# JonasGeiping/fullbatchtraining

Hardware: AMD Instinct MI355X
Metric: full-batch GD images/sec (ResNet-18 CIFAR-10 shaped, all chunks accumulated per step) (higher is better)
Workload: dtype bf16

## Files before the change

### fullbatchtraining_amd/csrc/conv_igemm.hip

```cpp
#include "common.h"
#include "profile.h"

#include "conv_params.h"

template <typename T, int BN_CO>
__global__ __launch_bounds__(256) void conv_igemm_kernel(const ConvParams p) {
    constexpr int EB = ET<T>::EB;
    constexpr int BKE = 128 / EB;
    constexpr int WROWS = BN_CO / 32;
    constexpr int FI = BN_CO / 32;
    constexpr int FJ = 4;
    constexpr int TILE_CHUNKS = (128 + BN_CO) * 8;
    __shared__ uint4 lds[2 * TILE_CHUNKS];

    const int tid = threadIdx.x, lane = tid & 63, wave = tid >> 6;
    const int wave_co = wave >> 1, wave_px = wave & 1;
    const int mblk = blockIdx.x, co_blk = blockIdx.y, cls = blockIdx.z;
    const int cpy = (p.os == 2) ? (cls >> 1) : 0, cpx = (p.os == 2) ? (cls & 1) : 0;
    const int chunk = tid & 7, lrow = tid >> 3;

    int a_img[4], a_y[4], a_x[4];
    const int qHW = p.qH * p.qW;
#pragma unroll
    for (int i = 0; i < 4; ++i) {
        const int m = mblk * 128 + lrow + 32 * i;
        if (m < p.M) {
            const int n = m / qHW, rem = m - n * qHW, qy = rem / p.qW, qx = rem - qy * p.qW;
            a_img[i] = n * p.Hs * p.Ws; a_y[i] = qy * p.ss; a_x[i] = qx * p.ss;
        } else {
            a_img[i] = 0; a_y[i] = -(1 << 28); a_x[i] = 0;
        }
    }
    const int first_img = (mblk * 128) / qHW;
    const char* wbase = p.wgt + (long long)(first_img / p.imgs_per_wset) * p.wset_stride_bytes;
    const int taps = p.R * p.S;
    const long long wrow_bytes = (long long)taps * p.Cs * EB;
    const char* wptr[WROWS];
#pragma unroll
    for (int i = 0; i < WROWS; ++i) wptr[i] = wbase + (long long)(co_blk * BN_CO + lrow + 32 * i) * wrow_bytes + chunk * 16;

    auto tap_valid = [&](int t, int& dy, int& dx) -> bool {
        const int r = t / p.S, s = t - r * p.S;
        if (p.mode == 0) { dy = r - p.pad; dx = s - p.pad; return true; }
        if (p.os == 1) { dy = p.pad - r; dx = p.pad - s; return true; }
        const int vy = cpy + p.pad - r, vx = cpx + p.pad - s;
        if ((vy & 1) || (vx & 1)) return false;
        dy = vy >> 1; dx = vx >> 1;
        return true;
    };
    const int kc = (p.Cs + BKE - 1) / BKE;
    int n_valid = 0;
    for (int t = 0; t < taps; ++t) { int dy, dx; n_valid += tap_valid(t, dy, dx) ? 1 : 0; }
    const int n_iter = n_valid * kc;

    uint4 ra[4], rw[WROWS];
    int cur_t = -1, cur_c = kc, cur_dy = 0, cur_dx = 0;
    auto advance = [&]() {
        if (++cur_c >= kc) {
            cur_c = 0;
            do { ++cur_t; } while (cur_t < taps && !tap_valid(cur_t, cur_dy, cur_dx));
        }
    };
    auto gload = [&]() {
        const int c0 = cur_c * BKE;
        const bool cvalid = c0 + chunk * ET<T>::VEC < p.Cs;
#pragma unroll
        for (int i = 0; i < 4; ++i) {
            const int sy = a_y[i] + cur_dy, sx = a_x[i] + cur_dx;
            const bool ok = cvalid && (unsigned)sy < (unsigned)p.Hs && (unsigned)sx < (unsigned)p.Ws;
            ra[i] = make_uint4(0, 0, 0, 0);
            if (ok) ra[i] = *(const uint4*)(p.src + ((long long)(a_img[i] + sy * p.Ws + sx) * p.Cs + c0) * EB + chunk * 16);
        }
#pragma unroll
        for (int i = 0; i < WROWS; ++i) {
            rw[i] = make_uint4(0, 0, 0, 0);
            if (cvalid) rw[i] = *(const uint4*)(wptr[i] + ((long long)cur_t * p.Cs + c0) * EB);
        }
    };
    auto lstore = [&](int buf) {
        uint4* base = lds + buf * TILE_CHUNKS;
#pragma unroll
        for (int i = 0; i < 4; ++i) { const int row = lrow + 32 * i; base[row * 8 + (chunk ^ (row & 7))] = ra[i]; }
#pragma unroll
        for (int i = 0; i < WROWS; ++i) { const int row = 128 + lrow + 32 * i; base[row * 8 + (chunk ^ (row & 7))] = rw[i]; }
    };

    f32x4_t acc[FI][FJ];
#pragma unroll
    for (int i = 0; i < FI; ++i)
#pragma unroll
        for (int j = 0; j < FJ; ++j) acc[i][j] = (f32x4_t){0.f, 0.f, 0.f, 0.f};

    if (n_iter > 0) {
        advance(); gload(); lstore(0);
        __syncthreads();
        for (int it = 0; it < n_iter; ++it) {
            const int buf = it & 1;
            const bool more = it + 1 < n_iter;
            if (more) { advance(); gload(); }
            const uint4* base = lds + buf * TILE_CHUNKS;
#pragma unroll
            for (int h = 0; h < 2; ++h) {
                const int pc = ((lane >> 4) + 4 * h) ^ (lane & 7);
                uint4 wf[FI], pf[FJ];
#pragma unroll
                for (int i = 0; i < FI; ++i) wf[i] = base[(128 + wave_co * (BN_CO / 2) + i * 16 + (lane & 15)) * 8 + pc];
#pragma unroll
                for (int j = 0; j < FJ; ++j) pf[j] = base[(wave_px * 64 + j * 16 + (lane & 15)) * 8 + pc];
#pragma unroll
                for (int i = 0; i < FI; ++i)
#pragma unroll
                    for (int j = 0; j < FJ; ++j) acc[i][j] = mma_chunk<T>(wf[i], pf[j], acc[i][j]);
            }
            if (more) lstore(buf ^ 1);
            __syncthreads();
        }
    }

    float ssum[FI][4], ssq[FI][4];
#pragma unroll
    for (int i = 0; i < FI; ++i)
#pragma unroll
        for (int r = 0; r < 4; ++r) { ssum[i][r] = 0.f; ssq[i][r] = 0.f; }
#pragma unroll
    for (int j = 0; j < FJ; ++j) {
        const int m = mblk * 128 + wave_px * 64 + j * 16 + (lane & 15);
        if (m < p.M) {
            const int n = m / qHW, rem = m - n * qHW, qy = rem / p.qW, qx = rem - qy * p.qW;
            const int oy = qy * p.os + cpy, ox = qx * p.os + cpx;
            const long long pix = ((long long)n * p.Hd + oy) * p.Wd + ox;
#pragma unroll
            for (int i = 0; i < FI; ++i) {
                const int co = co_blk * BN_CO + wave_co * (BN_CO / 2) + i * 16 + (lane >> 4) * 4;
                float v[4] = {acc[i][j][0], acc[i][j][1], acc[i][j][2], acc[i][j][3]};
                if (p.addend_mode == 1) {
                    const char* ap = p.addend + (pix * p.Cd + co) * EB;
                    if constexpr (EB == 4) { const float4 a = *(const float4*)ap; v[0] += a.x; v[1] += a.y; v[2] += a.z; v[3] += a.w; }
                    else { const uint2 a = *(const uint2*)ap; v[0] += __uint_as_float(a.x << 16); v[1] += __uint_as_float(a.x & 0xffff0000u);
                           v[2] += __uint_as_float(a.y << 16); v[3] += __uint_as_float(a.y & 0xffff0000u); }
                } else if (p.addend_mode == 2) {
                    const long long apix = ((long long)n * (p.Hd >> 1) + (oy >> 1)) * (p.Wd >> 1) + (ox >> 1);
                    const char* ap = p.addend + (apix * p.Cd + co) * EB;
                    if constexpr (EB == 4) { const float4 a = *(const float4*)ap; v[0] += 0.25f * a.x; v[1] += 0.25f * a.y; v[2] += 0.25f * a.z; v[3] += 0.25f * a.w; }
                    else { const uint2 a = *(const uint2*)ap; v[0] += 0.25f * __uint_as_float(a.x << 16); v[1] += 0.25f * __uint_as_float(a.x & 0xffff0000u);
                           v[2] += 0.25f * __uint_as_float(a.y << 16); v[3] += 0.25f * __uint_as_float(a.y & 0xffff0000u); }
                }
                char* dp = p.dst + (pix * p.Cd + co) * EB;
                if constexpr (EB == 4) *(float4*)dp = make_float4(v[0], v[1], v[2], v[3]);
                else *(uint2*)dp = make_uint2(pack_bf16x2(v[0], v[1]), pack_bf16x2(v[2], v[3]));
#pragma unroll
                for (int r = 0; r < 4; ++r) { ssum[i][r] += v[r]; ssq[i][r] += v[r] * v[r]; }
            }
        }
    }
    if (p.stat != nullptr) {
        float* red = (float*)lds;
        __syncthreads();
#pragma unroll
        for (int i = 0; i < FI; ++i)
#pragma unroll
            for (int r = 0; r < 4; ++r) {
                float a = ssum[i][r], b = ssq[i][r];
                a = row16_sum(a); b = row16_sum(b);
                if ((lane & 15) == 0) {
                    const int col = wave_co * (BN_CO / 2) + i * 16 + (lane >> 4) * 4 + r;
                    red[(wave_px * BN_CO + col) * 2] = a; red[(wave_px * BN_CO + col) * 2 + 1] = b;
                }
            }
        __syncthreads();
        if (tid < BN_CO) {
            const float a = red[tid * 2] + red[(BN_CO + tid) * 2];
            const float b = red[tid * 2 + 1] + red[(BN_CO + tid) * 2 + 1];
            const long long blk = (long long)cls * gridDim.x + mblk;
            p.stat[blk * p.Cd + co_blk * BN_CO + tid] = a;
            p.stat[((long long)p.n_mblocks + blk) * p.Cd + co_blk * BN_CO + tid] = b;
        }
    }
}

int fb_try_conv3x3_halo4(const fb_conv_args* a, hipStream_t st);
int fb_try_conv3x3_halo5(const fb_conv_args* a, hipStream_t st);
int fb_conv3x3_halo5_takes(const fb_conv_args* a);
int fb_try_conv3x3s2_dgrad_quad(const fb_conv_args* a, hipStream_t st);
int fb_try_conv1x1_k32(const fb_conv_args* a, hipStream_t st);
int fb_try_conv1x1_stream(const fb_conv_args* a, hipStream_t st);
int fb_try_conv1x1_gemm(const fb_conv_args* a, hipStream_t st);
int fb_try_conv1x1_pipe(const fb_conv_args* a, hipStream_t st);

int fb_conv1x1_pipe_takes(const fb_conv_args* a);
int fb_conv3x3_halo4_takes(const fb_conv_args* a);
int fb_conv1x1_gemm_takes(const fb_conv_args* a);
static int igemm_masked_addend_ok(const fb_conv_args* a) {
    if (getenv("FB_IGEMM_NO_MASK") != nullptr || a->mode != 1 || a->stride != 1 || a->bst_x) return 0;
    if (a->Cs % 32 != 0 || a->Cd % 64 != 0) return 0;
    static const bool v1 = getenv("FB_IGEMM_V1") != nullptr;
    if (v1) return 0;
    ConvParams p{};
    p.n_img = a->n_img; p.Hs = a->Hs; p.Ws = a->Ws; p.Cs = a->Cs; p.Hd = a->Hd; p.Wd = a->Wd; p.Cd = a->Cd; p.R = a->R; p.S = a->S;
    p.qH = a->Hd; p.qW = a->Wd;
    return fb_igemm_glds_fits(p, a->dtype);
}
extern "C" int32_t fb_conv_masked_addend_supported(const fb_conv_args* a) {
    if (!a || !a->addend || !a->addend_mask || a->addend_mode != 1) return 0;
    return fb_conv3x3_halo5_takes(a) || fb_conv1x1_pipe_takes(a) || fb_conv3x3_halo4_takes(a) || fb_conv1x1_gemm_takes(a) || igemm_masked_addend_ok(a);
}

extern "C" int32_t fb_conv_bwd_stat_supported(const fb_conv_args* a) {
    static const bool disabled = getenv("FB_DISABLE_FUSED_BWD_STAT") != nullptr;
    if (disabled || !a || !a->bst_x || !a->bst_mask || !a->stat_partial || a->mode != 1 || a->dtype != FB_BF16) return 0;
    if ((long long)a->n_img * a->Hd * a->Wd % 128 != 0) return 0;
    static const char* widths = getenv("FB_FUSED_BWD_STAT_W");
    if (widths) {
        char tag[8];
        snprintf(tag, sizeof(tag), "%d,", a->Wd);
        char list[64];
        snprintf(list, sizeof(list), "%s,", widths);
        if (!strstr(list, tag) || (a->Wd < 10 && list != strstr(list, tag) && *(strstr(list, tag) - 1) != ',')) return 0;
    }
    return fb_conv3x3_halo5_takes(a) || fb_conv3x3_halo4_takes(a);
}

template <typename T> static int launch_conv(const ConvParams& p, int classes, hipStream_t st) {
    const int mblocks = (p.M + 127) / 128;
    if (p.Cd % 128 == 0 && (long long)mblocks * (p.Cd / 128) * classes >= 512) {
        dim3 grid(mblocks, p.Cd / 128, classes);
        hipLaunchKernelGGL((conv_igemm_kernel<T, 128>), grid, dim3(256), 0, st, p);
    } else {
        dim3 grid(mblocks, p.Cd / 64, classes);
        hipLaunchKernelGGL((conv_igemm_kernel<T, 64>), grid, dim3(256), 0, st, p);
    }
    return 0;
}

extern "C" int fb_conv2d(const fb_conv_args* a, void* stream) {
    if (!a || !a->src || !a->wgt || !a->dst) FB_FAIL(FB_ERR_ARG, "fb_conv2d: null pointer");
    const int EB = a->dtype == FB_F32 ? 4 : 2;
    if (a->Cs % 32 != 0) FB_FAIL(FB_ERR_SHAPE, "fb_conv2d: Cs=%d must be a multiple of 32", a->Cs);
    if (a->Cd % 64 != 0) FB_FAIL(FB_ERR_SHAPE, "fb_conv2d: Cd=%d must be a multiple of 64", a->Cd);
    if (a->mode != 0 && a->mode != 1) FB_FAIL(FB_ERR_ARG, "fb_conv2d: mode %d", a->mode);
    if (a->addend_mask && !fb_conv_masked_addend_supported(a))
        FB_FAIL(FB_ERR_UNSUPPORTED, "fb_conv2d: addend_mask is not implemented for this shape (ask fb_conv_masked_addend_supported)");
    if (a->bst_x && !fb_conv_bwd_stat_supported(a))
        FB_FAIL(FB_ERR_UNSUPPORTED, "fb_conv2d: the fused BatchNorm-backward reduction is not implemented for this shape (ask fb_conv_bwd_stat_supported)");
    if (a->stride != 1 && a->stride != 2) FB_FAIL(FB_ERR_UNSUPPORTED, "fb_conv2d: stride %d", a->stride);
    ConvParams p;
    p.src = (const char*)a->src; p.wgt = (const char*)a->wgt; p.dst = (char*)a->dst; p.addend = (const char*)a->addend;
    p.stat = a->stat_partial;
    p.n_img = a->n_img; p.Hs = a->Hs; p.Ws = a->Ws; p.Cs = a->Cs; p.Hd = a->Hd; p.Wd = a->Wd; p.Cd = a->Cd;
    p.R = a->R; p.S = a->S; p.stride = a->stride; p.pad = a->pad; p.mode = a->mode;
    p.imgs_per_wset = a->imgs_per_wset > 0 ? a->imgs_per_wset : a->n_img;
    p.wset_stride_bytes = a->wset_stride * EB;
    p.addend_mode = a->addend ? a->addend_mode : 0;
    p.addend_mask = a->addend ? (const unsigned char*)a->addend_mask : nullptr;
    p.amax_src = a->dtype == FB_F32 ? a->amax_src : nullptr; p.amax_wgt = a->dtype == FB_F32 ? a->amax_wgt : nullptr;
    if ((p.amax_src == nullptr) != (p.amax_wgt == nullptr)) FB_FAIL(FB_ERR_ARG, "fb_conv2d: amax_src and amax_wgt go together");
    p.amax_imgs = a->amax_imgs > 0 ? a->amax_imgs : a->n_img;
    int classes = 1;
    if (a->mode == 0) {
        if (a->Hd != (a->Hs + 2 * a->pad - a->R) / a->stride + 1 || a->Wd != (a->Ws + 2 * a->pad - a->S) / a->stride + 1)
            FB_FAIL(FB_ERR_SHAPE, "fb_conv2d: fwd output %dx%d inconsistent with input %dx%d", a->Hd, a->Wd, a->Hs, a->Ws);
        p.qH = a->Hd; p.qW = a->Wd; p.os = 1; p.ss = a->stride;
    } else {
        if (a->Hs != (a->Hd + 2 * a->pad - a->R) / a->stride + 1 || a->Ws != (a->Wd + 2 * a->pad - a->S) / a->stride + 1)
            FB_FAIL(FB_ERR_SHAPE, "fb_conv2d: dgrad shapes inconsistent");
        if (a->stat_partial && !a->bst_x) FB_FAIL(FB_ERR_ARG, "fb_conv2d: statistics in mode 1 need bst_x / bst_mask");
        if (a->stride == 1) { p.qH = a->Hd; p.qW = a->Wd; p.os = 1; }
        else {
            if ((a->Hd & 1) || (a->Wd & 1)) FB_FAIL(FB_ERR_SHAPE, "fb_conv2d: stride-2 dgrad needs even input dims");
            p.qH = a->Hd / 2; p.qW = a->Wd / 2; p.os = 2; classes = 4;
        }
        p.ss = 1;
    }
    p.M = a->n_img * p.qH * p.qW;
    p.n_mblocks = ((p.M + 127) / 128) * classes;
    hipStream_t st = (hipStream_t)stream;
    const int32_t info[FB_PROF_INFO] = {a->n_img, a->Hs, a->Ws, a->Cs, a->Hd, a->Wd, a->Cd, a->R, a->stride,
                                        (a->addend ? a->addend_mode : 0) | (a->addend_mask ? 4 : 0) | (a->bst_x ? 8 : 0) | (a->dtype << 4), 0};
    const int prof = fb_prof_begin(a->mode == 0 ? FB_PROF_IGEMM_FWD : FB_PROF_IGEMM_DGRAD, st, info);
    static const bool v1 = getenv("FB_IGEMM_V1") != nullptr;
    int kernel = 0;
    if (fb_try_conv1x1_k32(a, st)) kernel = FB_K_CONV1X1_K32;
    else if ((a->mode == 0 || a->addend) && (a->Cs == 256 || a->Cs == 128) && fb_try_conv1x1_gemm(a, st)) kernel = FB_K_CONV1X1_GEMM;
    else if (fb_try_conv1x1_pipe(a, st)) kernel = FB_K_CONV1X1_PIPE;
    else if (fb_try_conv1x1_stream(a, st)) kernel = FB_K_CONV1X1_STREAM;
    else if (fb_try_conv1x1_gemm(a, st)) kernel = FB_K_CONV1X1_GEMM;
    else if (fb_try_conv3x3s2_dgrad_quad(a, st)) kernel = FB_K_S2_DGRAD_QUAD;
    else if (fb_try_conv3x3_halo5(a, st)) kernel = FB_K_HALO5;
    else if (fb_try_conv3x3_halo4(a, st)) kernel = FB_K_HALO4;
    else {
        p.zeros = nullptr;
        kernel = FB_K_IGEMM_GLDS;
        if (v1 || !fb_launch_igemm_glds(p, classes, a->dtype, st)) {
            if (p.addend_mask) FB_FAIL(FB_ERR_UNSUPPORTED, "fb_conv2d: the register-staged implicit GEMM does not apply addend_mask (tensor beyond 2^31 bytes per tile or FB_IGEMM_V1)");
            if (p.amax_src) FB_FAIL(FB_ERR_UNSUPPORTED, "fb_conv2d: the register-staged implicit GEMM has no fp16x2 path (tensor beyond 2^31 bytes or FB_IGEMM_V1)");
            if (a->dtype == FB_F32) launch_conv<float>(p, classes, st); else launch_conv<bf16_tag>(p, classes, st);
            kernel = FB_K_IGEMM_V1;
        }
    }
    fb_prof_kernel(prof, kernel);
    fb_prof_end(prof, st);
    FB_CHECK_LAUNCH("fb_conv2d");
    return FB_OK;
}
```

Baseline: 216,100.

## Add persistent halo-staged kernel for stride-2 3x3 forward conv 64->128

Adds a specialised persistent kernel for the ResNet-18 stride-2 3x3 forward convolution (32x32x64 to 16x16x128, bf16). Weights stay resident in registers, the input halo is loaded straight into LDS through buffer loads and double-buffered so the next tile prefetches during the current tile's MFMA work. BN statistics are fused into the epilogue. It replaces the generic implicit-GEMM path for this one layer shape, which can lower load traffic and launch overhead, at the cost of heavy register pressure and code tied to one shape. FB_K_S2_FWD is used but not defined in the shown code.

```diff
diff --git a/fullbatchtraining_amd/csrc/conv3x3s2_fwd.hip b/fullbatchtraining_amd/csrc/conv3x3s2_fwd.hip
--- /dev/null
+++ b/fullbatchtraining_amd/csrc/conv3x3s2_fwd.hip
@@ -0,0 +1,215 @@
+#include "common.h"
+
+#include <type_traits>
+
+struct S2FwdParams {
+    const char* src; const char* wgt; char* dst; float* stat;
+    int n_tiles;
+};
+
+namespace {
+template <int N> __device__ __forceinline__ void s2_wait_lgkmcnt() {
+    asm volatile("s_waitcnt lgkmcnt(%0)" ::"n"(N) : "memory");
+    __builtin_amdgcn_sched_barrier(0);
+}
+typedef __attribute__((ext_vector_type(4))) unsigned s2_u32x4;
+typedef __attribute__((ext_vector_type(2))) unsigned s2_u32x2;
+template <int OFF> __device__ __forceinline__ uint4 s2_read16(unsigned byte_addr) {
+    static_assert(OFF >= 0 && OFF < 65536, "ds offset");
+    s2_u32x4 v;
+    asm volatile("ds_read_b128 %0, %1 offset:%2" : "=v"(v) : "v"(byte_addr), "n"(OFF));
+    return make_uint4(v[0], v[1], v[2], v[3]);
+}
+template <int I, int N, typename F> __device__ __forceinline__ void s2_static_for(F&& f) {
+    if constexpr (I < N) { f(std::integral_constant<int, I>{}); s2_static_for<I + 1, N>(f); }
+}
+__device__ __forceinline__ int s2_xcd_remap(int b, int n) {
+    const int q = n >> 3, r = n & 7, xcd = b & 7, slot = b >> 3;
+    return (xcd < r ? xcd * (q + 1) : r * (q + 1) + (xcd - r) * q) + slot;
+}
+constexpr unsigned S2_OOB = 0x80000000u;
+constexpr int S2_W = 32;
+constexpr int S2_HY = 17, S2_EVEN = 17, S2_PITCH = 33;
+constexpr int S2_ROWS = S2_HY * S2_PITCH;
+constexpr int S2_NGRP = 72;
+constexpr int S2_HALO_BYTES = S2_NGRP * 1024;
+constexpr int S2_KH = S2_NGRP / 4;
+constexpr int S2_ROWB = S2_PITCH * 128;
+}
+
+__global__ __launch_bounds__(256) void conv3x3s2_fwd_kernel(const S2FwdParams p) {
+#if defined(__HIP_DEVICE_COMPILE__)
+    __shared__ __attribute__((aligned(16))) char lds[2 * S2_HALO_BYTES];
+
+    const int tid = threadIdx.x, lane = tid & 63;
+    const int wave = __builtin_amdgcn_readfirstlane(tid >> 6);
+    const int NB = gridDim.x;
+    const int lrow8 = lane >> 3, t = lane & 15, g = lane >> 4;
+    const unsigned lds0 = (unsigned)(size_t)(__attribute__((address_space(3))) char*)lds;
+
+    int L = s2_xcd_remap(blockIdx.x, NB);
+    if (L >= p.n_tiles) return;
+
+    unsigned voffH[S2_KH];
+    unsigned topbits = 0;
+#pragma unroll
+    for (int k = 0; k < S2_KH; ++k) {
+        const int e = (wave + 4 * k) * 8 + lrow8;
+        const int hy = e / S2_PITCH, rem = e - hy * S2_PITCH;
+        const int plane = rem >= S2_EVEN ? 1 : 0, idx = rem - plane * S2_EVEN, hx = 2 * idx + plane;
+        const bool ok = e < S2_ROWS && hx >= 1;
+        voffH[k] = ok ? (unsigned)((hy * S2_W + hx) * 128 + (((lane & 7) ^ (idx & 7)) * 16)) : S2_OOB;
+        topbits |= (hy == 0 ? 1u : 0u) << k;
+    }
+    auto halo_piece = [&](auto kc, int buf, int Ln) {
+        constexpr int K = decltype(kc)::value;
+        const int grp = wave + 4 * K;
+        const int n0 = Ln >> 1, hh = Ln & 1;
+        const long long origin = (((long long)n0 * S2_W + 16 * hh - 1) * S2_W - 1) * 128;
+        const __amdgpu_buffer_rsrc_t rA = __builtin_amdgcn_make_buffer_rsrc((void*)(p.src + origin), 0, (S2_HY * S2_W + 1) * 128, 0x00020000);
+        const unsigned v = (hh == 0 && ((topbits >> K) & 1u)) ? S2_OOB : voffH[K];
+        __builtin_amdgcn_raw_ptr_buffer_load_lds(rA, (__attribute__((address_space(3))) void*)(lds + buf * S2_HALO_BYTES + grp * 1024), 16, v, 0, 0, 0);
+    };
+    s2_static_for<0, S2_KH>([&](auto kc) { halo_piece(kc, 0, L); });
+
+    uint4 wf[9][2][2];
+#pragma unroll
+    for (int u = 0; u < 9; ++u)
+#pragma unroll
+        for (int h = 0; h < 2; ++h)
+#pragma unroll
+            for (int i = 0; i < 2; ++i)
+                wf[u][h][i] = *(const uint4*)(p.wgt + ((wave * 32 + 16 * i + t) * 9 + u) * 128 + (g + 4 * h) * 16);
+#pragma unroll
+    for (int u = 0; u < 9; ++u)
+#pragma unroll
+        for (int h = 0; h < 2; ++h)
+#pragma unroll
+            for (int i = 0; i < 2; ++i)
+                asm volatile("" : "+v"(wf[u][h][i].x), "+v"(wf[u][h][i].y), "+v"(wf[u][h][i].z), "+v"(wf[u][h][i].w));
+
+    unsigned pa[2][3][2];
+#pragma unroll
+    for (int bf = 0; bf < 2; ++bf)
+#pragma unroll
+        for (int s = 0; s < 3; ++s)
+#pragma unroll
+            for (int h = 0; h < 2; ++h)
+                pa[bf][s][h] = lds0 + bf * S2_HALO_BYTES + ((s & 1) * S2_EVEN + t + (s >> 1)) * 128 + (((g + 4 * h) ^ ((t + (s >> 1)) & 7)) * 16);
+    const int voffS = (t * 128 + wave * 32 + (g & 1) * 16 + (g >> 1) * 8) * 2;
+
+    s2_u32x4 outv[8];
+    float ssum[2][4], ssq[2][4];
+    auto store_tile = [&](const int Lp) {
+        const __amdgpu_buffer_rsrc_t rsrcD = __builtin_amdgcn_make_buffer_rsrc((void*)(p.dst + (long long)Lp * 128 * 256), 0, 128 * 256, 0x00020000);
+        s2_static_for<0, 8>([&](auto jc) {
+            constexpr int J = decltype(jc)::value;
+            __builtin_amdgcn_raw_buffer_store_b128(outv[J], rsrcD, voffS, J * 16 * 256, 0);
+            store_b128_guard(outv[J]);
+        });
+        if (p.stat != nullptr && t == 0) {
+#pragma unroll
+            for (int i = 0; i < 2; ++i) {
+                const int co = wave * 32 + i * 16 + g * 4;
+                *(float4*)(p.stat + (long long)Lp * 128 + co) = make_float4(ssum[i][0], ssum[i][1], ssum[i][2], ssum[i][3]);
+                *(float4*)(p.stat + ((long long)p.n_tiles + Lp) * 128 + co) = make_float4(ssq[i][0], ssq[i][1], ssq[i][2], ssq[i][3]);
+            }
+        }
+    };
+
+    auto tile = [&](auto bufc, const bool has_prev, const int L, const bool has_next) {
+        constexpr int BUF = decltype(bufc)::value;
+        asm volatile("s_waitcnt vmcnt(0)" ::: "memory");
+        __builtin_amdgcn_s_barrier();
+        if (has_prev) store_tile(L - NB);
+
+        f32x4_t acc[2][8];
+#pragma unroll
+        for (int i = 0; i < 2; ++i)
+#pragma unroll
+            for (int j = 0; j < 8; ++j) acc[i][j] = (f32x4_t){0.f, 0.f, 0.f, 0.f};
+
+        uint4 pf[2][8];
+        auto issue_reads = [&](auto sc) {
+            constexpr int S = decltype(sc)::value, U = S >> 1, H = S & 1, R = U / 3, SS = U % 3, SET = S & 1;
+            s2_static_for<0, 8>([&](auto jc) {
+                constexpr int J = decltype(jc)::value, HY = 2 * J + R;
+                if constexpr (HY < 15) pf[SET][J] = s2_read16<HY * S2_ROWB>(pa[BUF][SS][H]);
+                else pf[SET][J] = s2_read16<(HY - 8) * S2_ROWB>(pa[BUF][SS][H] + 8 * S2_ROWB);
+            });
+        };
+        issue_reads(std::integral_constant<int, 0>{});
+        s2_static_for<0, 18>([&](auto sc) {
+            constexpr int S = decltype(sc)::value, U = S >> 1, H = S & 1, SET = S & 1;
+            if constexpr (S + 1 < 18) {
+                issue_reads(std::integral_constant<int, S + 1>{});
+                s2_wait_lgkmcnt<8>();
+            } else {
+                s2_wait_lgkmcnt<0>();
+            }
+#pragma unroll
+            for (int j = 0; j < 8; ++j)
+#pragma unroll
+                for (int i = 0; i < 2; ++i) acc[i][j] = mma_chunk<bf16_tag>(wf[U][H][i], pf[SET][j], acc[i][j]);
+            if constexpr (S < S2_KH / 2) {
+                if (has_next) {
+                    halo_piece(std::integral_constant<int, 2 * S>{}, BUF ^ 1, L + NB);
+                    halo_piece(std::integral_constant<int, 2 * S + 1>{}, BUF ^ 1, L + NB);
+                }
+            }
+        });
+
+#pragma unroll
+        for (int i = 0; i < 2; ++i)
+#pragma unroll
+            for (int r = 0; r < 4; ++r) { ssum[i][r] = 0.f; ssq[i][r] = 0.f; }
+#pragma unroll
+        for (int j = 0; j < 8; ++j) {
+            unsigned pk[2][2];
+#pragma unroll
+            for (int i = 0; i < 2; ++i) {
+#pragma unroll
+                for (int r = 0; r < 4; ++r) { ssum[i][r] += acc[i][j][r]; ssq[i][r] += acc[i][j][r] * acc[i][j][r]; }
+                pk[i][0] = pack_bf16x2(acc[i][j][0], acc[i][j][1]); pk[i][1] = pack_bf16x2(acc[i][j][2], acc[i][j][3]);
+            }
+            const s2_u32x2 lo = __builtin_amdgcn_permlane16_swap(pk[0][0], pk[1][0], false, false);
+            const s2_u32x2 hi = __builtin_amdgcn_permlane16_swap(pk[0][1], pk[1][1], false, false);
+            outv[j] = (s2_u32x4){lo[0], hi[0], lo[1], hi[1]};
+        }
+#pragma unroll
+        for (int i = 0; i < 2; ++i)
+#pragma unroll
+            for (int r = 0; r < 4; ++r) { ssum[i][r] = row16_sum(ssum[i][r]); ssq[i][r] = row16_sum(ssq[i][r]); }
+    };
+
+    bool has_next = L + NB < p.n_tiles;
+    tile(std::integral_constant<int, 0>{}, false, L, has_next);
+    while (has_next) {
+        L += NB;
+        has_next = L + NB < p.n_tiles;
+        tile(std::integral_constant<int, 1>{}, true, L, has_next);
+        if (!has_next) break;
+        L += NB;
+        has_next = L + NB < p.n_tiles;
+        tile(std::integral_constant<int, 0>{}, true, L, has_next);
+    }
+    store_tile(L);
+#endif
+}
+
+int fb_try_conv3x3s2_fwd(const fb_conv_args* a, hipStream_t st) {
+    const char* sw = getenv("FB_S2_FWD");
+    if (sw && atoi(sw) == 0) return 0;
+    if (a->dtype != FB_BF16 || a->mode != 0) return 0;
+    if (a->R != 3 || a->S != 3 || a->stride != 2 || a->pad != 1) return 0;
+    if (a->Hs != 32 || a->Ws != 32 || a->Hd != 16 || a->Wd != 16 || a->Cs != 64 || a->Cd != 128) return 0;
+    if (a->imgs_per_wset > 0 && a->imgs_per_wset < a->n_img) return 0;
+    if (a->addend || a->addend_mask || a->bst_x || a->bst_mask || a->amax_src || a->amax_wgt) return 0;
+    if (a->n_img < 1 || a->n_img >= (1 << 24)) return 0;
+    S2FwdParams p;
+    p.src = (const char*)a->src; p.wgt = (const char*)a->wgt; p.dst = (char*)a->dst; p.stat = a->stat_partial;
+    p.n_tiles = a->n_img * 2;
+    const int n_cu = fb_persistent_cus();
+    hipLaunchKernelGGL(conv3x3s2_fwd_kernel, dim3(p.n_tiles < n_cu ? p.n_tiles : n_cu), dim3(256), 0, st, p);
+    return 1;
+}
diff --git a/fullbatchtraining_amd/csrc/conv_igemm.hip b/fullbatchtraining_amd/csrc/conv_igemm.hip
--- a/fullbatchtraining_amd/csrc/conv_igemm.hip
+++ b/fullbatchtraining_amd/csrc/conv_igemm.hip
@@ -182,6 +182,7 @@
 int fb_try_conv3x3_halo5(const fb_conv_args* a, hipStream_t st);
 int fb_conv3x3_halo5_takes(const fb_conv_args* a);
 int fb_try_conv3x3s2_dgrad_quad(const fb_conv_args* a, hipStream_t st);
+int fb_try_conv3x3s2_fwd(const fb_conv_args* a, hipStream_t st);
 int fb_try_conv1x1_k32(const fb_conv_args* a, hipStream_t st);
 int fb_try_conv1x1_stream(const fb_conv_args* a, hipStream_t st);
 int fb_try_conv1x1_gemm(const fb_conv_args* a, hipStream_t st);
@@ -287,6 +288,7 @@
     else if (fb_try_conv3x3s2_dgrad_quad(a, st)) kernel = FB_K_S2_DGRAD_QUAD;
     else if (fb_try_conv3x3_halo5(a, st)) kernel = FB_K_HALO5;
     else if (fb_try_conv3x3_halo4(a, st)) kernel = FB_K_HALO4;
+    else if (fb_try_conv3x3s2_fwd(a, st)) kernel = FB_K_S2_FWD;
     else {
         p.zeros = nullptr;
         kernel = FB_K_IGEMM_GLDS;
```

After: 217,100 (median of 6 runs). About the same (+0.5%).
